# dsteinberg/libcluster

Measured on AMD Instinct MI355X. Metric: E-step data-points/sec (full VBEM iteration: suff-stats + M-step + E-step), higher is better.
Workload: dtype f64

## Files before the change

### libcluster_amd/csrc/lc_kernels_suffstat.hip

```cpp
#include "lc_device.hpp"

#ifndef LC_SS_FEAT_MINK_ACTIVE
#define LC_SS_FEAT_MINK_ACTIVE 5
#endif
#ifndef LC_SS_FEAT_WIDTHS
#define LC_SS_FEAT_WIDTHS(DP) ((DP) >= 32 && (DP) <= 128)
#endif

namespace lck {

template <int NB>
struct SSAcc { static constexpr int N = NB * 3 + NB * (NB - 1) / 2 * 4; };

template <int NB>
__host__ __device__ constexpr bool ss_in_half(int half, int jbp, int jb) {
  if (half == 0) return true;
  const bool first = NB == 8   ? (jbp < 5 || (jbp == 5 && jb < 3))
                     : NB == 7 ? (jbp < 4 || (jbp == 4 && jb < 4))
                     : NB == 6 ? (jbp < 4 || (jbp == 4 && jb < 1))
                               : (jbp == 1 || jbp == 2);
  return first == (half == 1);
}
template <int PAN>
constexpr int ss_batch_rows() { return PAN == 2 ? 24 : SS_BR; }
// ... 670 lines not shown
#pragma unroll
        for (int c = 0; c < NQ; ++c) qa[c] = pq[QO + 4 * c];
#pragma unroll
        for (int st = 0; st < BR / 4; ++st) {
#pragma unroll
          for (int t = 0; t < NT; ++t) {
            const int cur = (st * NT + t) & 1, nxt = cur ^ 1;
            pp[t] = u[cur] * w[cur];
            if (t + 1 < NT) {
              u[nxt] = pu[t + 1][XO + st * 4 * LD];
              w[nxt] = pw[t + 1][XO + st * 4 * LD];
            } else if (st + 1 < BR / 4) {
              u[nxt] = pu[0][XO + (st + 1) * 4 * LD];
              w[nxt] = pw[0][XO + (st + 1) * 4 * LD];
            }
          }
          __builtin_amdgcn_sched_barrier(0);
#pragma unroll
          for (int c = 0; c < NQ; ++c) {
            if (on(st, c)) {
#pragma unroll
              for (int t = 0; t < NT; ++t) acc[t][c] = mfma4(qa[c], pp[t], acc[t][c]);
            }
            if (st + 1 < BR / 4) qa[c] = pq[QO + (st + 1) * 4 * QLD + 4 * c];
            __builtin_amdgcn_sched_barrier(0);
          }
        }
        return;
      }
      constexpr int G = SPECK ? ft_group_speck(DP) : ft_group(DP), TOT = (BR / 4) * NT;
      double qa[NQ], u[G], w[G], pp[G];
#pragma unroll
      for (int g = 0; g < G; ++g)
        if (g < TOT && g < NT) {
          u[g] = pu[g][XO];
          w[g] = pw[g][XO];
        }
#pragma unroll
      for (int c = 0; c < NQ; ++c) qa[c] = pq[QO + 4 * c];
#pragma unroll
      for (int st = 0; st < BR / 4; ++st) {
#pragma unroll
        for (int t0 = 0; t0 < NT; t0 += G) {
          const int ng = NT - t0 < G ? NT - t0 : G;
#pragma unroll
          for (int g = 0; g < G; ++g)
            if (g < ng) pp[g] = u[g] * w[g];
          const int nt0 = t0 + G < NT ? t0 + G : 0, nst = t0 + G < NT ? st : st + 1;
          if (nst < BR / 4) {
            const int nng = NT - nt0 < G ? NT - nt0 : G;
#pragma unroll
            for (int g = 0; g < G; ++g)
              if (g < nng) {
                u[g] = pu[nt0 + g][XO + nst * 4 * LD];
                w[g] = pw[nt0 + g][XO + nst * 4 * LD];
              }
          }
          const bool refill = nst != st && nst < BR / 4;
          __builtin_amdgcn_sched_barrier(0);
          if constexpr (SPECK) {
#pragma unroll
            for (int c4 = 0; c4 < NQ; c4 += 4) {
#pragma unroll
              for (int c = c4; c < c4 + 4 && c < NQ; ++c)
                if (on(st, c)) {
#pragma unroll
                  for (int g = 0; g < G; ++g)
                    if (g < ng) acc[t0 + g][c] = mfma4(qa[c], pp[g], acc[t0 + g][c]);
                }
              if (refill) {
#pragma unroll
                for (int c = c4; c < c4 + 4 && c < NQ; ++c) qa[c] = pq[QO + nst * 4 * QLD + 4 * c];
              }
              __builtin_amdgcn_sched_barrier(0);
            }
            continue;
          }
#pragma unroll
          for (int g = 0; g < G; ++g)
            if (g < ng) {
              if (refill && g + 1 == ng) {
#pragma unroll
                for (int c4 = 0; c4 < NQ; c4 += 4) {
#pragma unroll
                  for (int c = c4; c < c4 + 4 && c < NQ; ++c) acc[t0 + g][c] = mfma4(qa[c], pp[g], acc[t0 + g][c]);
#pragma unroll
                  for (int c = c4; c < c4 + 4 && c < NQ; ++c) qa[c] = pq[QO + nst * 4 * QLD + 4 * c];
                  __builtin_amdgcn_sched_barrier(0);
                }
              } else {
#pragma unroll
                for (int c = 0; c < NQ; ++c) acc[t0 + g][c] = mfma4(qa[c], pp[g], acc[t0 + g][c]);
              }
            }
          __builtin_amdgcn_sched_barrier(0);
        }
      }
      return;
    }
    double qa[ONEQ ? 1 : 2][NQ], u[2], w[2];
    u[0] = pu[0][XO];
    w[0] = pw[0][XO];
#pragma unroll
    for (int c = 0; c < NQ; ++c) qa[0][c] = pq[QO + 4 * c];
#pragma unroll
    for (int st = 0; st < BR / 4; ++st) {
#pragma unroll
      for (int t = 0; t < NT; ++t) {
        const int cur = (st * NT + t) & 1, nxt = cur ^ 1;
        const double p = u[cur] * w[cur];
        const bool refill = t + 1 == NT && st + 1 < BR / 4;
        if (t + 1 < NT) {
          u[nxt] = pu[t + 1][XO + st * 4 * LD];
          w[nxt] = pw[t + 1][XO + st * 4 * LD];
        } else if (st + 1 < BR / 4) {
          u[nxt] = pu[0][XO + (st + 1) * 4 * LD];
          w[nxt] = pw[0][XO + (st + 1) * 4 * LD];
          if constexpr (!ONEQ) {
#pragma unroll
            for (int c = 0; c < NQ; ++c) qa[(st + 1) & 1][c] = pq[QO + (st + 1) * 4 * QLD + 4 * c];
          }
        }
        __builtin_amdgcn_sched_barrier(0);
        if constexpr (ONEQ) {
#pragma unroll
          for (int c4 = 0; c4 < NQ; c4 += 4) {
#pragma unroll
            for (int c = c4; c < c4 + 4; ++c)
              if (on(st, c)) acc[t][c] = mfma4(qa[0][c], p, acc[t][c]);
            if (refill) {
#pragma unroll
              for (int c = c4; c < c4 + 4; ++c) qa[0][c] = pq[QO + (st + 1) * 4 * QLD + 4 * c];
            }
            __builtin_amdgcn_sched_barrier(0);
          }
        } else {
#pragma unroll
          for (int c = 0; c < NQ; ++c)
            if (on(st, c)) acc[t][c] = mfma4(qa[st & 1][c], p, acc[t][c]);
          __builtin_amdgcn_sched_barrier(0);
        }
      }
    }
  };
  for (int64_t b0 = r0; b0 < r1; b0 += 2 * BR) {
    const bool more1 = b0 + BR < r1, more2 = b0 + 2 * BR < r1;
    if (more1) gload(b0 + BR);
    if (!UNEVEN || nt == TPW) batch(std::integral_constant<int, 0>{}, std::integral_constant<int, TPW>{});
    else batch(std::integral_constant<int, 0>{}, std::integral_constant<int, TPWL>{});
    if (more1) lstore(1);
    __syncthreads();
    if (!more1) break;
    if (more2) gload(b0 + 2 * BR);
    if (!UNEVEN || nt == TPW) batch(std::integral_constant<int, 1>{}, std::integral_constant<int, TPW>{});
    else batch(std::integral_constant<int, 1>{}, std::integral_constant<int, TPWL>{});
    if (more2) lstore(0);
    __syncthreads();
  }

  const int64_t SS = 1 + (int64_t)DP + (int64_t)DP * DP;
  int sle = slice, T0e = 0, nte = 0;
  asm volatile("" : "+v"(sle));
  ft_deal(DP, DC, NQ, sle, wave, &T0e, &nte);
#pragma unroll
  for (int t = 0; t < TPW; ++t) {
    if (t >= nte) continue;
    const FtFeature f = ft_feature(DC, ONE, 16 * (T0e + t) + lo2 + 4 * blk);
    if (f.kind == FT_SPARE) continue;
#pragma unroll
    for (int c = 0; c < NQ; ++c) {
      const int kk = 4 * c + hi;
      if (kk >= KC) continue;
      double* out = a.partial + ((int64_t)chunk * a.KR + k0 + kk) * SS;
      const double v = acc[t][c];
      if (f.kind == FT_PRODUCT) {
        double* S = out + 1 + DP;
        S[(int64_t)f.u * DP + f.w] = v;
        S[(int64_t)f.w * DP + f.u] = v;
      } else if (f.kind == FT_LINEAR) {
        out[1 + f.u] = v;
      } else {
        out[0] = v;
      }
    }
  }
}

__global__ void __launch_bounds__(256) speck_probe_kernel(const double* qZ, int64_t ldq, int K, int64_t stride, int nsteps, int nq,
                                                           int nqp, int* active) {
  const int64_t t = (int64_t)blockIdx.x * 256 + threadIdx.x;
  const int c = (int)(t % nqp);
  unsigned rk = 0;
  if (t / nqp < nsteps && c < nq) {
    const int64_t row = 4 * stride * (t / nqp);
#pragma unroll
    for (int i = 0; i < 4; ++i) {
      const int k = 4 * c + i;
      if (k < K) {
        const double2* qp = reinterpret_cast<const double2*>(qZ + (int64_t)k * ldq + row);
        const double2 v0 = qp[0], v1 = qp[1];
        rk |= (!(v0.x < SPECK_TAU) ? 1u : 0u) | (!(v0.y < SPECK_TAU) ? 2u : 0u) | (!(v1.x < SPECK_TAU) ? 4u : 0u) |
              (!(v1.y < SPECK_TAU) ? 8u : 0u);
      }
    }
  }
  const int lane = threadIdx.x & 63;
  const unsigned long long b = __ballot(rk != 0);
  if (lane == 0 && b != 0) atomicAdd(active, __popcll(b));
  if (nqp <= 64) {
    const unsigned long long grp = (nqp == 64 ? ~0ull : ((1ull << nqp) - 1ull)) << (lane & ~(nqp - 1));
    int single = 0;
#pragma unroll
    for (int i = 0; i < 4; ++i) {
      const unsigned long long br = __ballot((rk >> i) & 1u);
      single += __popcll(__ballot(c == 0 && __popcll(br & grp) == 1));
    }
    if (lane == 0 && single != 0) atomicAdd(active + 1, single);
  }
}
hipError_t launch_speck_probe(const double* qZ, int64_t ldq, int K, int64_t NP, int* active, int64_t* pairs, hipStream_t stream,
                              int64_t* rows) {
  const int64_t steps = NP / 4;
  *pairs = 0;
  if (rows) *rows = 0;
  if (hipError_t e = hipMemsetAsync(active, 0, 2 * sizeof(int), stream); e != hipSuccess) return e;
  if (steps < 1 || K < 1) return hipSuccess;
  const int nsteps = (int)(steps < SPECK_PROBE_STEPS ? steps : SPECK_PROBE_STEPS), nq = (K + 3) / 4;
  const int64_t stride = steps / nsteps;
  int nqp = 1;
  while (nqp < nq) nqp *= 2;
  *pairs = (int64_t)nsteps * nq;
  if (rows && nqp <= 64) *rows = 4 * (int64_t)nsteps;
  hipLaunchKernelGGL(speck_probe_kernel, dim3((unsigned)(((int64_t)nsteps * nqp + 255) / 256)), dim3(256), 0, stream, qZ, ldq, K, stride,
                     nsteps, nq, nqp, active);
  return hipGetLastError();
}

template <int DP, int DC, int NQ, bool SPECK>
static hipError_t launch_ss_feat_i(const SuffstatLaunch& b, hipStream_t stream) {
  constexpr int BR = ft_batch_rows(DP), LD = lds_row_stride(DP);
  const size_t shmem = (size_t)(2 * BR * LD + 2 * BR * ft_qld(NQ)) * sizeof(double);
  auto kern = suffstat_feat_kernel<DP, DC, NQ, SPECK>;
  static LdsGrant grant;
  if (hipError_t e = grant_dynamic_lds(reinterpret_cast<const void*>(kern), shmem, grant); e != hipSuccess) return e;
  hipLaunchKernelGGL(kern, dim3((unsigned)(b.nchunks * ft_nslice(DP, DC, NQ))), dim3(64 * ft_waves(DP)), shmem, stream, b);
  return hipGetLastError();
}
template <int DP, int DC, int NQ>
static hipError_t launch_ss_feat_q(const SuffstatLaunch& b, hipStream_t stream) {
  return b.speck_skip ? launch_ss_feat_i<DP, DC, NQ, true>(b, stream) : launch_ss_feat_i<DP, DC, NQ, false>(b, stream);
}
template <int DP, int DC>
static hipError_t launch_ss_feat_d(const SuffstatLaunch& a, hipStream_t stream) {
  SuffstatLaunch b = a;
  const int range = ft_range(DP, a.K);
  for (int k0 = 0; k0 < a.K; k0 += range) {
    b.klast0 = k0;
    const int nq = ((a.K - k0 < range ? a.K - k0 : range) + 3) / 4;
    hipError_t e = hipErrorInvalidValue;
    switch (ft_instance_quads(nq)) {
      case 2: e = launch_ss_feat_q<DP, DC, 2>(b, stream); break;
      case 4: e = launch_ss_feat_q<DP, DC, 4>(b, stream); break;
      case 5: e = launch_ss_feat_q<DP, DC, 5>(b, stream); break;
      case 6: e = launch_ss_feat_q<DP, DC, 6>(b, stream); break;
      case 7: e = launch_ss_feat_q<DP, DC, 7>(b, stream); break;
      case 8: e = launch_ss_feat_q<DP, DC, 8>(b, stream); break;
      case 16:
        if constexpr (DP == 128) e = launch_ss_feat_q<DP, DC, 16>(b, stream);
        break;
    }
    if (e != hipSuccess) return e;
  }
  return hipSuccess;
}
template <int DP>
static hipError_t launch_ss_feat_w(const SuffstatLaunch& a, hipStream_t stream) {
  if constexpr (DP <= 48) {
    if (a.DC == DP - 4) return launch_ss_feat_d<DP, DP - 4>(a, stream);
    if (a.DC == DP - 12) return launch_ss_feat_d<DP, DP - 12>(a, stream);
  }
  if (a.DC == DP - 8) return launch_ss_feat_d<DP, DP - 8>(a, stream);
  if (a.DC != 0 && a.DC != DP) return hipErrorInvalidValue;
  return launch_ss_feat_d<DP, DP>(a, stream);
}
static hipError_t launch_ss_feat(const SuffstatLaunch& a, hipStream_t stream) {
  switch (a.DP) {
    case 32: return launch_ss_feat_w<32>(a, stream);
    case 48: return launch_ss_feat_w<48>(a, stream);
    case 64: return launch_ss_feat_w<64>(a, stream);
    case 80: return launch_ss_feat_w<80>(a, stream);
    case 96: return launch_ss_feat_w<96>(a, stream);
    case 112: return launch_ss_feat_w<112>(a, stream);
    case 128: return launch_ss_feat_w<128>(a, stream);
  }
  return hipErrorInvalidValue;
}

#ifndef LC_FT_SPECK_LISTS
#define LC_FT_SPECK_LISTS 1
#endif
#ifndef LC_FTL_BR
#define LC_FTL_BR 48
#endif
bool speck_lists_enabled() { return LC_FT_SPECK_LISTS != 0; }
#ifndef LC_FT_LIST_SHARE64
#define LC_FT_LIST_SHARE64 58
#endif
bool speck_probe_says_lists(int64_t single, int64_t rows) { return rows > 0 && 64 * single >= (int64_t)LC_FT_LIST_SHARE64 * rows; }
bool suffstat_list_instance(int DP, int DC) { return DP == 64 && (DC == 0 || DC == 64 || DC == 56); }

template <typename IT>
__global__ void __launch_bounds__(256) ss_list_build_kernel(const double* __restrict__ qZ, int64_t ldq, int K, int64_t NP,
                                                             int64_t chunk_rows, int nq, int* __restrict__ lens, IT* __restrict__ ent) {
  __shared__ int wcnt[2][32][4];
  const int chunk = blockIdx.x, tid = threadIdx.x, lane = tid & 63, wave = tid >> 6;
  const int64_t r0 = (int64_t)chunk * chunk_rows;
  const int64_t r1 = (r0 + chunk_rows) < NP ? (r0 + chunk_rows) : NP;
  if (r0 >= r1) {
    for (int c = tid; c < nq; c += 256) lens[(int64_t)chunk * nq + c] = 0;
    return;
  }
  for (int q0 = 0; q0 < nq; q0 += 32) {
    const int nqg = nq - q0 < 32 ? nq - q0 : 32;
    int base = 0, par = 0;
    for (int64_t t0 = r0; t0 < r1; t0 += 256, par ^= 1) {
      const int64_t row = t0 + tid;
      const bool valid = row < r1;
      const double* qr = qZ + (valid ? row : r1 - 1);
      unsigned m = 0;
      for (int c8 = 0; c8 < nqg; c8 += 8) {
        double v[32];
#pragma unroll
        for (int i = 0; i < 32; ++i) {
          const int k = 4 * (q0 + c8) + i;
          v[i] = qr[(int64_t)(k < K ? k : K - 1) * ldq];
        }
#pragma unroll
        for (int i = 0; i < 32; ++i) {
          const int k = 4 * (q0 + c8) + i;
          if (valid && k < K && !(v[i] < SPECK_TAU)) m |= 1u << (c8 + i / 4);
        }
      }
      int mycnt = 0;
      for (int c = 0; c < nqg; ++c) {
        const unsigned long long bal = __ballot((m >> c) & 1u);
        if (lane == c) mycnt = __popcll(bal);
      }
      if (lane < nqg) wcnt[par][lane][wave] = mycnt;
      __syncthreads();
      int mybase = 0;
      if (lane < nqg) {
        int tot = 0, before = 0;
#pragma unroll
        for (int w = 0; w < 4; ++w) {
          const int n = wcnt[par][lane][w];
          before += w < wave ? n : 0;
          tot += n;
        }
        mybase = base + before;
        base += tot;
      }
      for (int c = 0; c < nqg; ++c) {
        const unsigned long long bal = __ballot((m >> c) & 1u);
        const int at = __shfl(mybase, c) + (int)__builtin_amdgcn_mbcnt_hi((unsigned)(bal >> 32), __builtin_amdgcn_mbcnt_lo((unsigned)bal, 0u));
        if ((m >> c) & 1u) ent[((int64_t)chunk * nq + q0 + c) * chunk_rows + at] = (IT)(row - r0);
      }
    }
    if (wave == 0 && lane < nqg) lens[(int64_t)chunk * nq + q0 + lane] = base;
    __syncthreads();
  }
}

template <int DP, int DC, typename IT>
__global__ void __launch_bounds__(512, 2) suffstat_list_kernel(SuffstatLaunch a, const int* __restrict__ lens, const IT* __restrict__ ent,
                                                                int nq) {
  static_assert(DC % 4 == 0 && DC <= DP && DC > DP - 16, "active width");
  constexpr int NTHR = 512, BR = LC_FTL_BR, LD = lds_row_stride(DP), QLD = 4, XBUF = BR * LD, QBUF = BR * QLD;
  constexpr int ONE = DP, NT = ftl_tpw(DC);
  constexpr int TPR = DP / 2, RPP = NTHR / TPR, NPRE = BR / RPP;
  static_assert(LD > DP && NTHR % TPR == 0 && BR % RPP == 0 && BR % 4 == 0 && 4 * BR <= NTHR, "staging");
  static_assert((XBUF + (BR - 4) * LD + LD) * 8 <= 65536, "fragment reads: one address register per tile, the rest immediate");
  extern __shared__ __attribute__((aligned(16))) double lds[];
  double* xbuf = lds;
  double* qbuf = lds + 2 * XBUF;
  const int tid = threadIdx.x, lane = tid & 63, wave = tid >> 6;
  const int hi = lane >> 4, blk = (lane >> 2) & 3, lo2 = lane & 3;
  const int chunk = blockIdx.x / nq, quad = blockIdx.x % nq;
  const int64_t r0 = (int64_t)chunk * a.chunk_rows;
  const int len = lens[blockIdx.x];
  const IT* li = ent + (int64_t)blockIdx.x * a.chunk_rows;
  constexpr int NW = ftl_nw(DC);
  const double* pu[NT];
  const double* pw[NW];
#pragma unroll
  for (int t = 0; t < NT; ++t) {
    const FtlFeature f = ftl_feature(DC, ONE, wave, t, lo2 + 4 * blk);
    pu[t] = xbuf + hi * LD + f.u;
    int ow = hi * LD + f.w;
    if constexpr (ftl_shared(DC)) asm volatile("" : "+v"(ow));
    pw[ftl_wi(DC, t)] = xbuf + ow;
  }
  double acc[NT];
#pragma unroll
  for (int t = 0; t < NT; ++t) acc[t] = 0.0;

  const int xr0 = tid / TPR, xc2 = tid % TPR, qrow = tid / 4, qcl = tid % 4;
  const bool qthr = tid < 4 * BR;
  const int kq = 4 * quad + qcl;
  const double* qcol = a.qZ + (int64_t)(kq < a.K ? kq : a.K - 1) * a.ldq + r0;
  int xi[NPRE], qi = -1;
  double pre[NPRE][2], qpre = 0.0;
  auto iload = [&](int p0) {
#pragma unroll
    for (int i = 0; i < NPRE; ++i) {
      const int p = p0 + xr0 + i * RPP;
      xi[i] = p < len ? (int)li[p] : -1;
    }
    qi = qthr && p0 + qrow < len ? (int)li[p0 + qrow] : -1;
  };
  auto gload = [&]() {
#pragma unroll
    for (int i = 0; i < NPRE; ++i) {
      const double2 v = *reinterpret_cast<const double2*>(a.X + (r0 + (xi[i] < 0 ? 0 : xi[i])) * DP + 2 * xc2);
      pre[i][0] = xi[i] < 0 ? 0.0 : v.x;
      pre[i][1] = xi[i] < 0 ? 0.0 : v.y;
    }
    const double q = qcol[qi < 0 ? 0 : qi];
    qpre = qi < 0 || kq >= a.K ? 0.0 : q;
  };
  auto lstore = [&](int buf) {
#pragma unroll
    for (int i = 0; i < NPRE; ++i)
      *reinterpret_cast<double2*>(xbuf + buf * XBUF + (xr0 + i * RPP) * LD + 2 * xc2) = make_double2(pre[i][0], pre[i][1]);
    if (qthr) qbuf[buf * QBUF + qrow * QLD + qcl] = qpre;
  };
  if (tid < 2 * BR) xbuf[(tid / BR) * XBUF + (tid % BR) * LD + ONE] = 1.0;
  if (len > 0) {
    iload(0);
    gload();
    iload(BR);
    lstore(0);
  }
  __syncthreads();
  const double* pq = qbuf + hi * QLD + lo2;
  auto batch = [&](auto bsel) {
    constexpr int B = decltype(bsel)::value, XO = B * XBUF, QO = B * QBUF;
    double uf[NT], wf[NW], pp[NT];
#pragma unroll
    for (int t = 0; t < NT; ++t) uf[t] = pu[t][XO];
#pragma unroll
    for (int i = 0; i < NW; ++i) wf[i] = pw[i][XO];
    double qa = pq[QO];
    if constexpr (ftl_shared(DC)) __builtin_amdgcn_sched_barrier(0);
#pragma unroll
    for (int st = 0; st < BR / 4; ++st) {
#pragma unroll
      for (int t = 0; t < NT; ++t) pp[t] = uf[t] * wf[ftl_wi(DC, t)];
      const double qc = qa;
      if (st + 1 < BR / 4) {
#pragma unroll
        for (int t = 0; t < NT; ++t) uf[t] = pu[t][XO + (st + 1) * 4 * LD];
#pragma unroll
        for (int i = 0; i < NW; ++i) wf[i] = pw[i][XO + (st + 1) * 4 * LD];
        qa = pq[QO + (st + 1) * 4 * QLD];
      }
      __builtin_amdgcn_sched_barrier(0);
#pragma unroll
      for (int t = 0; t < NT; ++t) acc[t] = mfma4(qc, pp[t], acc[t]);
      __builtin_amdgcn_sched_barrier(0);
    }
  };
  for (int p0 = 0; p0 < len; p0 += 2 * BR) {
    const bool more1 = p0 + BR < len, more2 = p0 + 2 * BR < len;
    if (more1) {
      gload();
      iload(p0 + 2 * BR);
    }
    batch(std::integral_constant<int, 0>{});
    if (more1) lstore(1);
    __syncthreads();
    if (!more1) break;
    if (more2) {
      gload();
      iload(p0 + 3 * BR);
    }
    batch(std::integral_constant<int, 1>{});
    if (more2) lstore(0);
    __syncthreads();
  }

  const int64_t SS = 1 + (int64_t)DP + (int64_t)DP * DP;
  int wv = wave;
  asm volatile("" : "+v"(wv));
  const int kk = 4 * quad + hi;
  if (kk >= a.K) return;
  double* out = a.partial + ((int64_t)chunk * a.KR + kk) * SS;
#pragma unroll
  for (int t = 0; t < NT; ++t) {
    const FtlFeature f = ftl_feature(DC, ONE, wv, t, lo2 + 4 * blk);
    if (f.kind == FT_SPARE) continue;
    const double v = acc[t];
    if (f.kind == FT_PRODUCT) {
      double* S = out + 1 + DP;
      S[(int64_t)f.u * DP + f.w] = v;
      S[(int64_t)f.w * DP + f.u] = v;
    } else if (f.kind == FT_LINEAR) {
      out[1 + f.u] = v;
    } else {
      out[0] = v;
    }
  }
}

static hipError_t ss_list_check(const SuffstatLaunch& a, const SuffstatPlan& p, const void* lists, size_t bytes, SsListLayout* lay) {
  if (a.K <= 0 || p.nchunks <= 0 || !lists || !a.qZ || !a.X) return hipErrorInvalidValue;
  if (p.route != SS_FEAT || a.mode != SS_DENSE || a.smask || a.items || p.extra != 0) return hipErrorInvalidValue;
  if (a.nchunks != p.nchunks || a.chunk_rows != p.chunk_rows || a.KR != p.KR || a.KR != a.K) return hipErrorInvalidValue;
  if (!suffstat_list_instance(a.DP, a.DC)) return hipErrorInvalidValue;
  if (a.chunk_rows < 4 || a.chunk_rows % 4 || a.chunk_rows > (int64_t)1 << 30 || (int64_t)a.nchunks * a.chunk_rows < a.NP) return hipErrorInvalidValue;
  *lay = ss_list_layout(a.nchunks, a.chunk_rows, a.K);
  if ((int64_t)a.nchunks * lay->nq > (int64_t)1 << 30 || bytes < lay->bytes) return hipErrorInvalidValue;
  return hipSuccess;
}
hipError_t launch_suffstat_list_build(const SuffstatLaunch& a, const SuffstatPlan& p, void* lists, size_t bytes, hipStream_t stream) {
  SsListLayout lay;
  if (hipError_t e = ss_list_check(a, p, lists, bytes, &lay); e != hipSuccess) return e;
  int* lens = static_cast<int*>(lists);
  void* ent = static_cast<char*>(lists) + lay.ent_off;
  if (lay.wide)
    hipLaunchKernelGGL(ss_list_build_kernel<unsigned>, dim3((unsigned)a.nchunks), dim3(256), 0, stream, a.qZ, a.ldq, a.K, a.NP,
                       a.chunk_rows, lay.nq, lens, static_cast<unsigned*>(ent));
  else
    hipLaunchKernelGGL(ss_list_build_kernel<unsigned short>, dim3((unsigned)a.nchunks), dim3(256), 0, stream, a.qZ, a.ldq, a.K, a.NP,
                       a.chunk_rows, lay.nq, lens, static_cast<unsigned short*>(ent));
  return hipGetLastError();
}
template <int DP, int DC, typename IT>
static hipError_t launch_ss_list_i(const SuffstatLaunch& a, const SsListLayout& lay, const void* lists, hipStream_t stream) {
  constexpr int BR = LC_FTL_BR;
  const size_t shmem = (size_t)(2 * BR * lds_row_stride(DP) + 2 * BR * 4) * sizeof(double);
  auto kern = suffstat_list_kernel<DP, DC, IT>;
  static LdsGrant grant;
  if (hipError_t e = grant_dynamic_lds(reinterpret_cast<const void*>(kern), shmem, grant); e != hipSuccess) return e;
  hipLaunchKernelGGL(kern, dim3((unsigned)(a.nchunks * lay.nq)), dim3(512), shmem, stream, a, static_cast<const int*>(lists),
                     reinterpret_cast<const IT*>(static_cast<const char*>(lists) + lay.ent_off), lay.nq);
  return hipGetLastError();
}
hipError_t launch_suffstat_lists(const SuffstatLaunch& a, const SuffstatPlan& p, void* lists, size_t bytes, hipStream_t stream) {
  SsListLayout lay;
  if (hipError_t e = ss_list_check(a, p, lists, bytes, &lay); e != hipSuccess) return e;
  if (hipError_t e = launch_suffstat_list_build(a, p, lists, bytes, stream); e != hipSuccess) return e;
  const bool narrow = a.DC == 56;
  if (lay.wide) return narrow ? launch_ss_list_i<64, 56, unsigned>(a, lay, lists, stream) : launch_ss_list_i<64, 64, unsigned>(a, lay, lists, stream);
  return narrow ? launch_ss_list_i<64, 56, unsigned short>(a, lay, lists, stream)
                : launch_ss_list_i<64, 64, unsigned short>(a, lay, lists, stream);
}

struct SqItem {
  int kind, ia, ja;
};
__host__ __device__ constexpr int sq_items(int DC) { return (DC / 4) * (DC / 4 + 1) / 2 + DC / 4 + 1; }
__host__ __device__ constexpr SqItem sq_item(int DC, int n) {
  for (int ja = 0; ja < DC / 4; ++ja) {
    if (n <= ja) return SqItem{0, n, ja};
    n -= ja + 1;
    if (n == 0) return SqItem{1, 0, ja};
    n -= 1;
  }
  return SqItem{2, 0, 0};
}
__host__ __device__ constexpr int sq_part_lo(int DC, int NPART, int p) { return (sq_items(DC) * p + NPART - 1) / NPART; }
__host__ __device__ constexpr int sq_part_max(int DC, int NPART) {
  int m = 0;
  for (int p = 0; p < NPART; ++p) {
    const int n = sq_part_lo(DC, NPART, p + 1) - sq_part_lo(DC, NPART, p);
    m = n > m ? n : m;
  }
  return m;
}
constexpr int SQ_BR = 32, SQ_QLD = 18;
inline int sq_npart(int DP, int K) {
  const int nq = (K + 3) / 4;
  if (DP > 48) return 4;
  return nq == 2 ? 2 : nq == 4 ? (DP <= 32 ? 1 : 2) : 4;
}
inline int sq_nslice(int DP, int K) { return (((K + 3) / 4) * sq_npart(DP, K) + 3) / 4; }
inline bool ss_quad_eligible(int DP, int K) {
  static const int mode = test_switch("LC_SS_QUAD") ? atoi(test_switch("LC_SS_QUAD")) : -1;
  if (mode == 0 || DP < 32 || DP > 64 || K < 1 || K > 16) return false;
  if (mode == 1) return true;
  return K >= 3;
}
template <int DP, int DC, int NPART>
__global__ void __launch_bounds__(256, 2) suffstat_quad_kernel(SuffstatLaunch a) {
  static_assert(DC % 4 == 0 && DC <= DP && DC > DP - 16, "active width");
  constexpr int NT = DC / 4, BR = SQ_BR, LD = lds_row_stride(DP), QLD = SQ_QLD, XBUF = BR * LD, QBUF = BR * QLD, NTHR = 256;
  constexpr int NACC = sq_part_max(DC, NPART);
  extern __shared__ __attribute__((aligned(16))) double lds[];
  double* xbuf = lds;
  double* qbuf = lds + 2 * XBUF;
  const int tid = threadIdx.x, lane = tid & 63, wave = tid >> 6;
  const int hi = lane >> 4, blk = (lane >> 2) & 3, lo2 = lane & 3;
  const int K = a.K, NQ = (K + 3) / 4;
  int chunk, slice;
  {
    const int nslice = a.nslice, nchunks = a.nchunks, b = blockIdx.x, full = (nchunks / 8) * 8;
    if (b < full * nslice) {
      const int xcd = b & 7, seq = b >> 3;
      chunk = (seq / nslice) * 8 + xcd;
      slice = seq % nslice;
    } else {
      const int t = b - full * nslice;
      chunk = full + t / nslice;
      slice = t % nslice;
    }
  }
  const int64_t r0 = (int64_t)chunk * a.chunk_rows;
  const int64_t r1 = (r0 + a.chunk_rows) < a.NP ? (r0 + a.chunk_rows) : a.NP;
  const int unit = slice * 4 + wave, quad = unit / NPART, part = unit % NPART;
  const bool busy = quad < NQ;

  constexpr int TPR = DP / 2, NV2 = BR * TPR, NPRE = (NV2 + NTHR - 1) / NTHR;
  double pre[NPRE][2], qpre[4];
  const int qcl = tid % 16, qrq = tid / 16;
  const bool qthr = qrq < BR / 4;
  auto gload = [&](int64_t b0) {
#pragma unroll
    for (int i = 0; i < NPRE; ++i) {
      const int idx = tid + i * NTHR;
      const int row = idx / TPR, c2 = idx % TPR;
      double2 v = make_double2(0.0, 0.0);
      if (row < BR && b0 + row < r1) v = *reinterpret_cast<const double2*>(a.X + (b0 + row) * DP + 2 * c2);
      pre[i][0] = v.x;
      pre[i][1] = v.y;
    }
    const int64_t qrow = b0 + 4 * qrq;
#pragma unroll
    for (int i = 0; i < 4; ++i) qpre[i] = 0.0;
    if (qthr && qcl < K && qrow < r1) {
      const double2* qp = reinterpret_cast<const double2*>(a.qZ + (int64_t)qcl * a.ldq + qrow);
      const double2 v0 = qp[0], v1 = qp[1];
      qpre[0] = v0.x, qpre[1] = v0.y, qpre[2] = v1.x, qpre[3] = v1.y;
    }
  };
  auto lstore = [&](int buf) {
#pragma unroll
    for (int i = 0; i < NPRE; ++i) {
      const int idx = tid + i * NTHR;
      const int row = idx / TPR, c2 = idx % TPR;
      if (row < BR) *reinterpret_cast<double2*>(xbuf + buf * XBUF + row * LD + 2 * c2) = make_double2(pre[i][0], pre[i][1]);
    }
    if (qthr) {
#pragma unroll
      for (int i = 0; i < 4; ++i) qbuf[buf * QBUF + (4 * qrq + i) * QLD + qcl] = qpre[i];
    }
  };

  double acc[NACC];
#pragma unroll
  for (int i = 0; i < NACC; ++i) acc[i] = 0.0;
  const double* px = xbuf + hi * LD + lo2;
  const double* pq = qbuf + hi * QLD + 4 * (busy ? quad : 0) + blk;

  auto batch = [&](auto bsel, auto psel) {
    constexpr int B = decltype(bsel)::value, P = decltype(psel)::value, XO = B * XBUF, QO = B * QBUF;
    constexpr int LO = sq_part_lo(DC, NPART, P), HI = sq_part_lo(DC, NPART, P + 1);
    constexpr int JA0 = sq_item(DC, LO).kind == 2 ? NT - 1 : sq_item(DC, LO).ja;
    constexpr int JA1 = sq_item(DC, HI - 1).kind == 2 ? NT - 1 : sq_item(DC, HI - 1).ja;
    double xa[2][JA1 + 1], qa[2];
#pragma unroll
    for (int t = 0; t <= JA1; ++t) xa[0][t] = px[XO + 4 * t];
    qa[0] = pq[QO];
#pragma unroll
    for (int st = 0; st < BR / 4; ++st) {
      const int cur = st & 1, nxt = cur ^ 1;
      double pr[JA1 - JA0 + 1];
#pragma unroll
      for (int j = JA0; j <= JA1; ++j) pr[j - JA0] = qa[cur] * xa[cur][j];
      if (st + 1 < BR / 4) {
#pragma unroll
        for (int t = 0; t <= JA1; ++t) xa[nxt][t] = px[XO + (st + 1) * 4 * LD + 4 * t];
        qa[nxt] = pq[QO + (st + 1) * 4 * QLD];
      }
      static_for<HI - LO>([&](auto ic) {
        constexpr SqItem it = sq_item(DC, LO + ic);
        if constexpr (it.kind == 1) acc[ic] += pr[it.ja - JA0];
        else if constexpr (it.kind == 2) acc[ic] += qa[cur];
      });
      __builtin_amdgcn_sched_barrier(0);
      static_for<HI - LO>([&](auto ic) {
        constexpr SqItem it = sq_item(DC, LO + ic);
        if constexpr (it.kind == 0) acc[ic] = mfma4(xa[cur][it.ia], pr[it.ja - JA0], acc[ic]);
      });
      __builtin_amdgcn_sched_barrier(0);
    }
  };
  auto run = [&](auto psel) {
    if (r0 < r1) {
      gload(r0);
      lstore(0);
    }
    __syncthreads();
    for (int64_t b0 = r0; b0 < r1; b0 += 2 * BR) {
      const bool more1 = b0 + BR < r1, more2 = b0 + 2 * BR < r1;
      if (more1) gload(b0 + BR);
      if (busy) batch(std::integral_constant<int, 0>{}, psel);
      if (more1) lstore(1);
      __syncthreads();
      if (!more1) break;
      if (more2) gload(b0 + 2 * BR);
      if (busy) batch(std::integral_constant<int, 1>{}, psel);
      if (more2) lstore(0);
      __syncthreads();
    }
    if (!busy) return;
    constexpr int P = decltype(psel)::value, LO = sq_part_lo(DC, NPART, P), HI = sq_part_lo(DC, NPART, P + 1);
    const int kk = 4 * quad + blk;
    if (kk >= K) return;
    const int64_t SS = 1 + (int64_t)DP + (int64_t)DP * DP;
    double* out = a.partial + ((int64_t)chunk * a.KR + kk) * SS;
    double* S = out + 1 + DP;
    static_for<HI - LO>([&](auto ic) {
      constexpr SqItem it = sq_item(DC, LO + ic);
      const double v = acc[ic];
      if constexpr (it.kind == 0) {
        const int gi = 4 * it.ia + hi, gj = 4 * it.ja + lo2;
        if constexpr (it.ia == it.ja) {
          if (hi >= lo2) S[(int64_t)gi * DP + gj] = v;
          if (hi > lo2) S[(int64_t)gj * DP + gi] = v;
        } else {
          S[(int64_t)gi * DP + gj] = v;
          S[(int64_t)gj * DP + gi] = v;
        }
      } else if constexpr (it.kind == 1) {
        const double t = sum_over_hi(v);
        if (hi == 0) out[1 + 4 * it.ja + lo2] = t;
      } else {
        const double t = sum_over_hi(v);
        if (hi == 0 && lo2 == 0) out[0] = t;
      }
    });
  };
  if constexpr (NPART == 1) {
    run(std::integral_constant<int, 0>{});
  } else if constexpr (NPART == 2) {
    if (part == 0) run(std::integral_constant<int, 0>{});
    else run(std::integral_constant<int, 1>{});
  } else {
    static_assert(NPART == 4, "parts per quad");
    if (part == 0) run(std::integral_constant<int, 0>{});
    else if (part == 1) run(std::integral_constant<int, 1>{});
    else if (part == 2) run(std::integral_constant<int, 2>{});
    else run(std::integral_constant<int, 3>{});
  }
}

template <int DP, int DC, class F>
static hipError_t sq_instance_d(int K, F& f) {
  const int np = sq_npart(DP, K);
  using dp = std::integral_constant<int, DP>;
  using dc = std::integral_constant<int, DC>;
  if constexpr (DP <= 32) {
    if (np == 1) return f(dp{}, dc{}, std::integral_constant<int, 1>{});
  }
  if constexpr (DP <= 48) {
    if (np == 2) return f(dp{}, dc{}, std::integral_constant<int, 2>{});
  }
  return np == 4 ? f(dp{}, dc{}, std::integral_constant<int, 4>{}) : hipErrorInvalidValue;
}
template <int DP, class F>
static hipError_t sq_instance_w(int DC, int K, F& f) {
  if constexpr (DP <= 48) {
    if (DC == DP - 4) return sq_instance_d<DP, DP - 4>(K, f);
    if (DC == DP - 12) return sq_instance_d<DP, DP - 12>(K, f);
  }
  if (DC == DP - 8) return sq_instance_d<DP, DP - 8>(K, f);
  if (DC != 0 && DC != DP) return hipErrorInvalidValue;
  return sq_instance_d<DP, DP>(K, f);
}
template <class F>
static hipError_t sq_instance(int DP, int DC, int K, F f) {
  switch (DP) {
    case 32: return sq_instance_w<32>(DC, K, f);
    case 48: return sq_instance_w<48>(DC, K, f);
    case 64: return sq_instance_w<64>(DC, K, f);
  }
  return hipErrorInvalidValue;
}
static size_t sq_lds_bytes(int DP) { return (size_t)(2 * SQ_BR * lds_row_stride(DP) + 2 * SQ_BR * SQ_QLD) * sizeof(double); }
static hipError_t launch_ss_quad(const SuffstatLaunch& a, hipStream_t stream) {
  return sq_instance(a.DP, a.DC, a.K, [&](auto dp, auto dc, auto np) {
// ... 247 lines not shown
```

Baseline: 377.9 million.

## Interleave next-stage LDS fragment reads between MFMAs in suffstat list kernel

In the list-based suffstat kernel, the LDS reads for the next stage's fragments are now spread across the MFMA sequence (a compile-time schedule via ftl_read) instead of issued as one block before the MFMAs. The aim is to hide LDS latency behind matrix ops and reduce register pressure spikes. The double-buffer loop also becomes unconditional, always loading and storing, with validity masking moved from load time to LDS store time, which removes branches but may issue redundant global loads past the end of the list.

Result: faster. 386.8 million (median of 6 runs) (+2.4%).

```diff
diff --git a/libcluster_amd/csrc/lc_kernels_suffstat.hip b/libcluster_amd/csrc/lc_kernels_suffstat.hip
--- a/libcluster_amd/csrc/lc_kernels_suffstat.hip
+++ b/libcluster_amd/csrc/lc_kernels_suffstat.hip
@@ -996,6 +996,21 @@
 #ifndef LC_FTL_BR
 #define LC_FTL_BR 48
 #endif
+#ifndef LC_FTL_SPREAD
+#define LC_FTL_SPREAD 12
+#endif
+__host__ __device__ constexpr int ftl_read(int DC, int r) {
+  int n = 0;
+  for (int t = 0; t < ftl_tpw(DC); ++t) {
+    if (t == 0 || ftl_wi(DC, t) != ftl_wi(DC, t - 1)) {
+      if (n == r) return -1 - ftl_wi(DC, t);
+      ++n;
+    }
+    if (n == r) return t;
+    ++n;
+  }
+  return ftl_tpw(DC);
+}
 bool speck_lists_enabled() { return LC_FT_SPECK_LISTS != 0; }
 #ifndef LC_FT_LIST_SHARE64
 #define LC_FT_LIST_SHARE64 58
@@ -1084,6 +1099,7 @@
   const int len = lens[blockIdx.x];
   const IT* li = ent + (int64_t)blockIdx.x * a.chunk_rows;
   constexpr int NW = ftl_nw(DC);
+  constexpr int NRD = NT + NW + 1, SPREAD = LC_FTL_SPREAD < 0 ? 0 : LC_FTL_SPREAD < NT ? LC_FTL_SPREAD : NT;
   const double* pu[NT];
   const double* pw[NW];
 #pragma unroll
@@ -1104,6 +1120,8 @@
   const double* qcol = a.qZ + (int64_t)(kq < a.K ? kq : a.K - 1) * a.ldq + r0;
   int xi[NPRE], qi = -1;
   double pre[NPRE][2], qpre = 0.0;
+  constexpr bool LATE = SPREAD != 0;
+  bool xok[NPRE], qok = false;
   auto iload = [&](int p0) {
 #pragma unroll
     for (int i = 0; i < NPRE; ++i) {
@@ -1116,17 +1134,20 @@
 #pragma unroll
     for (int i = 0; i < NPRE; ++i) {
       const double2 v = *reinterpret_cast<const double2*>(a.X + (r0 + (xi[i] < 0 ? 0 : xi[i])) * DP + 2 * xc2);
-      pre[i][0] = xi[i] < 0 ? 0.0 : v.x;
-      pre[i][1] = xi[i] < 0 ? 0.0 : v.y;
+      xok[i] = xi[i] >= 0;
+      pre[i][0] = LATE || xok[i] ? v.x : 0.0;
+      pre[i][1] = LATE || xok[i] ? v.y : 0.0;
     }
     const double q = qcol[qi < 0 ? 0 : qi];
-    qpre = qi < 0 || kq >= a.K ? 0.0 : q;
+    qok = qi >= 0 && kq < a.K;
+    qpre = LATE || qok ? q : 0.0;
   };
   auto lstore = [&](int buf) {
 #pragma unroll
     for (int i = 0; i < NPRE; ++i)
-      *reinterpret_cast<double2*>(xbuf + buf * XBUF + (xr0 + i * RPP) * LD + 2 * xc2) = make_double2(pre[i][0], pre[i][1]);
-    if (qthr) qbuf[buf * QBUF + qrow * QLD + qcl] = qpre;
+      *reinterpret_cast<double2*>(xbuf + buf * XBUF + (xr0 + i * RPP) * LD + 2 * xc2) =
+          make_double2(!LATE || xok[i] ? pre[i][0] : 0.0, !LATE || xok[i] ? pre[i][1] : 0.0);
+    if (qthr) qbuf[buf * QBUF + qrow * QLD + qcl] = !LATE || qok ? qpre : 0.0;
   };
   if (tid < 2 * BR) xbuf[(tid / BR) * XBUF + (tid % BR) * LD + ONE] = 1.0;
   if (len > 0) {
@@ -1151,36 +1172,73 @@
 #pragma unroll
       for (int t = 0; t < NT; ++t) pp[t] = uf[t] * wf[ftl_wi(DC, t)];
       const double qc = qa;
-      if (st + 1 < BR / 4) {
-#pragma unroll
-        for (int t = 0; t < NT; ++t) uf[t] = pu[t][XO + (st + 1) * 4 * LD];
-#pragma unroll
-        for (int i = 0; i < NW; ++i) wf[i] = pw[i][XO + (st + 1) * 4 * LD];
-        qa = pq[QO + (st + 1) * 4 * QLD];
-      }
-      __builtin_amdgcn_sched_barrier(0);
-#pragma unroll
-      for (int t = 0; t < NT; ++t) acc[t] = mfma4(qc, pp[t], acc[t]);
-      __builtin_amdgcn_sched_barrier(0);
+      if constexpr (SPREAD == 0) {
+        if (st + 1 < BR / 4) {
+#pragma unroll
+          for (int t = 0; t < NT; ++t) uf[t] = pu[t][XO + (st + 1) * 4 * LD];
+#pragma unroll
+          for (int i = 0; i < NW; ++i) wf[i] = pw[i][XO + (st + 1) * 4 * LD];
+          qa = pq[QO + (st + 1) * 4 * QLD];
+        }
+        __builtin_amdgcn_sched_barrier(0);
+#pragma unroll
+        for (int t = 0; t < NT; ++t) acc[t] = mfma4(qc, pp[t], acc[t]);
+        __builtin_amdgcn_sched_barrier(0);
+      } else {
+        __builtin_amdgcn_sched_barrier(0);
+#pragma unroll
+        for (int t = 0; t < NT; ++t) {
+          acc[t] = mfma4(qc, pp[t], acc[t]);
+          if (st + 1 < BR / 4 && t < SPREAD) {
+#pragma unroll
+            for (int r = t * NRD / SPREAD; r < (t + 1) * NRD / SPREAD; ++r) {
+              const int what = ftl_read(DC, r);
+              if (what == NT)
+                qa = pq[QO + (st + 1) * 4 * QLD];
+              else if (what >= 0)
+                uf[what] = pu[what][XO + (st + 1) * 4 * LD];
+              else
+                wf[-1 - what] = pw[-1 - what][XO + (st + 1) * 4 * LD];
+            }
+          }
+          __builtin_amdgcn_sched_barrier(0);
+        }
+      }
     }
   };
-  for (int p0 = 0; p0 < len; p0 += 2 * BR) {
-    const bool more1 = p0 + BR < len, more2 = p0 + 2 * BR < len;
-    if (more1) {
+  if constexpr (LATE) {
+    for (int p0 = 0; p0 < len; p0 += 2 * BR) {
       gload();
       iload(p0 + 2 * BR);
-    }
-    batch(std::integral_constant<int, 0>{});
-    if (more1) lstore(1);
-    __syncthreads();
-    if (!more1) break;
-    if (more2) {
+      batch(std::integral_constant<int, 0>{});
+      lstore(1);
+      __syncthreads();
+      if (p0 + BR >= len) break;
       gload();
       iload(p0 + 3 * BR);
-    }
-    batch(std::integral_constant<int, 1>{});
-    if (more2) lstore(0);
-    __syncthreads();
+      batch(std::integral_constant<int, 1>{});
+      lstore(0);
+      __syncthreads();
+    }
+  } else {
+    for (int p0 = 0; p0 < len; p0 += 2 * BR) {
+      const bool more1 = p0 + BR < len, more2 = p0 + 2 * BR < len;
+      if (more1) {
+        gload();
+        iload(p0 + 2 * BR);
+      }
+      batch(std::integral_constant<int, 0>{});
+      if (more1) lstore(1);
+      __syncthreads();
+      if (!more1) break;
+      if (more2) {
+        gload();
+        iload(p0 + 3 * BR);
+      }
+      batch(std::integral_constant<int, 1>{});
+      if (more2) lstore(0);
+      __syncthreads();
+    }
   }
 
   const int64_t SS = 1 + (int64_t)DP + (int64_t)DP * DP;
```
